# I-Mihara/BioDemuX.jl

Hardware: AMD Instinct MI355X
Metric: reads/s demultiplexed (150 bp, 96 barcodes, :semiglobal) at 1/2/4/8 MI355X (higher is better)
Workload: dtype i32

## Files before the change

### biodemux.jl_amd/csrc/bdx_sweep_col.h

```cpp
#pragma once
#include <stdint.h>

#if defined(__HIPCC__)
#define BDX_COL_FN __host__ __device__ __forceinline__
#else
#define BDX_COL_FN inline
#endif

#define BDX_COL_FIELD_MASK 0x1C1C1C1Cu

BDX_COL_FN uint32_t bdx_col_junk(const int nv) { return nv >= 8 ? 0u : (nv <= 0 ? 0x44444444u : (0x44444444u << (4 * nv))); }

BDX_COL_FN void bdx_col_fields(const uint32_t A, const uint32_t mask, uint32_t &ev, uint32_t &od) {
    ev = (A << 2) & mask;
    od = (A >> 2) & mask;
}
BDX_COL_FN uint32_t bdx_col_field(const uint32_t ev, const uint32_t od, const int k) { return (((k & 1) ? od : ev) >> (8 * (k >> 1))) & 0xFFu; }

BDX_COL_FN int bdx_col_score_carry(uint32_t &Ph, uint32_t &Mh, int score) {
#if defined(__has_builtin) && __has_builtin(__builtin_addc)
    uint32_t cp, cm;
    Ph = __builtin_addc(Ph, Ph, 0u, &cp);
    Mh = __builtin_addc(Mh, Mh, 0u, &cm);
#else
    const uint64_t p2 = (uint64_t)Ph + Ph, m2 = (uint64_t)Mh + Mh;
    const uint32_t cp = (uint32_t)(p2 >> 32), cm = (uint32_t)(m2 >> 32);
    Ph = (uint32_t)p2;
    Mh = (uint32_t)m2;
#endif
    score += (int)cp;
    score -= (int)cm;
    return score;
}

BDX_COL_FN uint32_t bdx_col_dbl(uint32_t x) {
#if defined(__HIP_DEVICE_COMPILE__)
    asm("v_add_u32 %0, %0, %0" : "+v"(x));
    return x;
#else
    return x + x;
#endif
}

template <bool TRACK, bool ADD = false>
BDX_COL_FN uint32_t sweep_step(const uint32_t Eq, uint32_t &Pv, uint32_t &Mv, int &score, int &best) {
    const uint32_t Xv = Eq | Mv;
    const uint32_t ep = Eq & Pv;
    const uint32_t Xh = ((ep + Pv) ^ Pv) | Eq;
    uint32_t Ph = Mv | ~(Xh | Pv);
    uint32_t Mh = Pv & Xh;
    if (TRACK) {
        score = bdx_col_score_carry(Ph, Mh, score);
    } else {
        Ph = ADD ? bdx_col_dbl(Ph) : Ph + Ph;
        Mh = ADD ? bdx_col_dbl(Mh) : Mh + Mh;
    }
    Pv = Mh | ~(Xv | Ph);
    Mv = Ph & Xv;
    if (TRACK) best = score < best ? score : best;
    return ep;
}
```

### biodemux.jl_amd/csrc/bdx_wave_kernel.h

```cpp
#pragma once

#include <atomic>

#include <cstdio>
#include <cstdlib>

#include "bdx_core.h"
#include "bdx_read_index.h"
#include "bdx_sweep_col.h"

#define BDX_BAD_PLAN() (getenv("BDX_TRACE_LAUNCH") ? (void)fprintf(stderr, "[bdx] launch refused at %s:%d\n", __FILE__, __LINE__) : (void)0, hipErrorInvalidValue)

namespace {

struct WaveArgs {
    double max_error_rate, min_delta;
    int counts_stride2;
    uint32_t rix_mul;
    const uint8_t *seq;
    const long long *off;
    long long n_reads;
    BdxDevOut out;
    unsigned long long *counts;
    int hist_entries;
// ... 31 lines not shown
    int vps, vps_inv;
    int max_len;
    int win_sfe, win_so, win_efe, win_eo;
    int cpr;
    int cpr_inv;
    int hq_cap, sq_cap;
    int ngroups;
    int scan_gpr, scan_gpr_inv;
    int cand_area;
    int ranged;
    BdxDevPass dpass[2];
    const uint32_t *idmap;
    const unsigned int *n_dev;
    uint32_t req;
    int dbg;
};

typedef const __attribute__((address_space(4))) WaveArgs *KArgs;
__device__ __forceinline__ KArgs kargs() {
    uint64_t p = (uint64_t)(uintptr_t)__builtin_amdgcn_kernarg_segment_ptr();
    asm volatile("" : "+s"(p));
    return (KArgs)(uintptr_t)p;
}

enum : uint32_t {
    REQ_BC1 = 1u, REQ_BC2 = 2u, REQ_KS = 4u, REQ_KE = 8u, REQ_PSTART = 16u, REQ_PEND = 32u, REQ_PRAW = 64u, REQ_PBC = 128u,
    REQ_PSCORE = 256u, REQ_PDELTA = 512u, REQ_COUNTS = 1024u,
    REQ_TIER = 2048u, REQ_DELTA = 4096u,
    REQ_PASS = REQ_PSTART | REQ_PEND | REQ_PRAW | REQ_PBC | REQ_PSCORE | REQ_PDELTA
};

#ifdef BDX_TUNING
#define BDX_DBG(bit) (a.dbg & (bit))
#else
#define BDX_DBG(bit) 0
#endif

typedef unsigned int u32x2 __attribute__((ext_vector_type(2)));
typedef unsigned int u32x3 __attribute__((ext_vector_type(3)));

#define WAVE_SYNC()                                          \
    do {                                                     \
        __builtin_amdgcn_fence(__ATOMIC_RELEASE, "wavefront"); \
        __builtin_amdgcn_wave_barrier();                     \
        __builtin_amdgcn_fence(__ATOMIC_ACQUIRE, "wavefront"); \
    } while (0)

template <bool EXACT, bool DOT>
__device__ __forceinline__ void pack16(const u32x4 v, uint32_t &p2, uint32_t &nlo, uint32_t &nhi, uint32_t &sad, const uint32_t m7 = 0x07070707u,
                                       const uint32_t m3 = 0x03030303u) {
    constexpr uint32_t CODE_LO = 0x03020100u, CODE_HI = 0x04040404u;
    constexpr uint32_t EXP_LO = 0x47544341u , EXP_HI = 0x4E000000u ;
    uint32_t u[4], t2[4];
#pragma unroll
    for (int w = 0; w < 4; ++w) {
        const uint32_t x = v[w];
        const uint32_t sel = (x >> 1) & m7;
        uint32_t n4 = __builtin_amdgcn_perm(CODE_HI, CODE_LO, sel);
        const uint32_t e = __builtin_amdgcn_perm(EXP_HI, EXP_LO, sel);
        if (EXACT) {
            const uint32_t d = x ^ e;
            const uint32_t y = (((d & 0x7F7F7F7Fu) + 0x7F7F7F7Fu) | d) & 0x80808080u;
            const uint32_t m = (y >> 7) * 0xFFu;
            n4 = (n4 & ~m) | (m & 0x04040404u);
        } else {
            sad = __builtin_amdgcn_sad_u8(x, e, sad);
        }
        u[w] = n4 | (n4 >> 4);
        if (DOT) {
            t2[w] = __builtin_amdgcn_udot4(sel & m3, 0x40100401u, 0u, false);
        } else {
            const uint32_t t6 = (x & 0x06060606u) << 5;
            const uint32_t a = t6 | (t6 << 6);
            t2[w] = a | (a << 12);
        }
    }
    nlo = __builtin_amdgcn_perm(u[1], u[0], 0x06040200u);
    nhi = __builtin_amdgcn_perm(u[3], u[2], 0x06040200u);
    const uint32_t lo = __builtin_amdgcn_perm(t2[1], t2[0], DOT ? 0x0C0C0400u : 0x0C0C0703u);
    const uint32_t hi = __builtin_amdgcn_perm(t2[3], t2[2], DOT ? 0x04000C0Cu : 0x07030C0Cu);
    p2 = lo | hi;
}

__device__ __forceinline__ void lds_read8(uint32_t (&d)[8], const uint32_t (&addr)[8]) {
#pragma unroll
    for (int i = 0; i < 8; ++i) asm volatile("ds_read_b32 %0, %1" : "=v"(d[i]) : "v"(addr[i]) : "memory");
}
__device__ __forceinline__ void lds_wait8(uint32_t (&d)[8]) {
    asm volatile("s_waitcnt lgkmcnt(0)"
                 : "+v"(d[0]), "+v"(d[1]), "+v"(d[2]), "+v"(d[3]), "+v"(d[4]), "+v"(d[5]), "+v"(d[6]), "+v"(d[7])
                 :
                 : "memory");
}

__device__ __forceinline__ int wave_cols(const int rem) {
    int x = 0;
#pragma unroll
    for (int bit = 16; bit > 0; bit >>= 1)
        if (__builtin_amdgcn_ballot_w64(rem > x + bit)) x += bit;
    return x + 1;
}

template <int TF, int TRACKW, bool COLS>
__device__ __forceinline__ void sweep_block(const uint32_t A0, const uint32_t A1, const uint32_t A2, const uint32_t A3,
                                            const uint32_t pbase, uint32_t &Pv, uint32_t &Mv, int &score, int &best, const int kk1,
                                            uint32_t &inm, uint32_t &inm2, const int nc) {
    const int ngr = COLS ? (nc + 7) >> 3 : nc;
    const uint32_t A[4] = {A0, A1, A2, A3};
    uint32_t Eq[2][8];
    uint32_t fmask = BDX_COL_FIELD_MASK;
    if (COLS) asm("" : "+v"(fmask));
    const auto issue = [&](const int h) __attribute__((always_inline)) {
        uint32_t addr[8];
        if (COLS) {
            uint32_t ev, od;
            bdx_col_fields(A[h], fmask, ev, od);
            asm volatile("" : "+v"(ev), "+v"(od));
#pragma unroll
            for (int jj = 0; jj < 8; ++jj) addr[jj] = pbase + bdx_col_field(ev, od, jj);
        } else {
#pragma unroll
            for (int jj = 0; jj < 8; ++jj) addr[jj] = pbase + (__builtin_amdgcn_ubfe(A[h], 4 * jj, 3) << 2);
        }
        lds_read8(Eq[h & 1], addr);
    };
    issue(0);
    inm = 0u;
    inm2 = 0u;
#pragma unroll
    for (int h = 0; h < 4; ++h) {
        if (h >= ngr) break;
        lds_wait8(Eq[h & 1]);
        if (h < 3 && h + 1 < ngr) issue(h + 1);
#pragma unroll
        for (int jj = 0; jj < 8; ++jj) {
            const int j = 8 * h + jj;
            if (COLS && jj > 0 && j >= nc) break;
            if (j < TF) {
                sweep_step<false, COLS>(Eq[h & 1][jj], Pv, Mv, score, best);
            } else {
                if (j == TF && TF > 0) score = __builtin_popcount(Pv) - __builtin_popcount(Mv);
                const int best_before = best;
                const uint32_t ep = sweep_step<true, COLS>(Eq[h & 1][jj], Pv, Mv, score, best);
                if (TRACKW == 1) inm = __builtin_amdgcn_alignbit(inm, (uint32_t)(score - kk1), 31);
                if (TRACKW >= 2) inm = __builtin_amdgcn_alignbit(inm, (uint32_t)(score - best_before), 31);
                if (TRACKW >= 3) inm2 = __builtin_amdgcn_alignbit(inm2, ep, 31);
            }
        }
    }
    const int ran = COLS ? nc : 8 * ngr;
    if (TRACKW && ran < 32) inm <<= 32 - ran;
    if (TRACKW >= 3 && ran < 32) inm2 <<= 32 - ran;
}

template <bool REVA>
__device__ __forceinline__ void anchored_block(const uint32_t A0, const uint32_t A1, const uint32_t A2, const uint32_t A3, const uint32_t pbase,
                                               const uint32_t rows, const uint32_t lowbit, uint32_t &Pv, uint32_t &Mv, int &score, const int d,
                                               uint32_t &eqm, uint32_t &inm2, const int ngr) {
    const uint32_t A[4] = {A0, A1, A2, A3};
    uint32_t Eq[2][8];
    const auto issue = [&](const int h) __attribute__((always_inline)) {
        uint32_t addr[8];
#pragma unroll
        for (int jj = 0; jj < 8; ++jj) addr[jj] = pbase + (__builtin_amdgcn_ubfe(A[h], 4 * jj, 3) << 2);
        lds_read8(Eq[h & 1], addr);
    };
// ... 54 lines not shown
    const uint32_t req = a.req;
    static_assert(!WINM || (!PAIRS && !SPLIT && KEND == 0 && GEN), "window mode: the non-split single-seed kernel");
    constexpr bool SCAT = PAIRS || WINM;
    constexpr bool CARRY = PAIRS && !SPLIT && !MG && KB <= 4;
    const uint32_t idmask = (CARRY && a.carry_ent != nullptr) ? 0x3FFFFFFFu : 0xFFFFFFFFu;
    const long long n_reads = (SCAT && a.n_dev) ? (long long)(unsigned int)__builtin_amdgcn_readfirstlane((int)*a.n_dev) : a.n_reads;

    size_t o = 0;
    auto take = [&](size_t bytes) -> LDS unsigned char * {
        LDS unsigned char *p = smem + o;
        o = (o + bytes + 31) & ~(size_t)31;
        return p;
    };
    LDS unsigned char *bm = take((size_t)a.bm_bytes);
    LDS uint16_t *rnk = (LDS uint16_t *)take(PAIRS ? 0 : (size_t)a.bm_bytes / 2);
    LDS uint32_t *ent = (LDS uint32_t *)take((size_t)a.n_ent * 4);
    LDS uint32_t *peq = (LDS uint32_t *)take((size_t)B * 36);
    LDS uint32_t *peqr = (LDS uint32_t *)take(KREV ? (size_t)B * 36 : 0);
    LDS uint32_t *meta = (LDS uint32_t *)take((size_t)B * 4);
    LDS uint32_t *settle = (LDS uint32_t *)take((size_t)B * 4);
    LDS int *hist = (LDS int *)take((size_t)a.hist_entries * 4);
    LDS unsigned char *wbase = smem + o + (size_t)wv * (size_t)a.per_wave;
    constexpr int O_FB = 0;
    constexpr int O_RID = O_FB + ((RW + 1) * 4 + 15) / 16 * 16;
    constexpr int O_RMK = O_RID + NREC * 4;
    constexpr int O_SLOTS = O_RMK + NREC * 4;
    constexpr int O_SCNT = O_SLOTS + RW * 16;
    constexpr int O_FLAG = O_SCNT + RW * 4;
    constexpr int O_WCL1 = O_FLAG + RW * 4;
    constexpr int O_LBUF = O_WCL1 + RW * 4;
    constexpr int O_RL = O_LBUF + 64 * 4;
    constexpr int O_GID = O_RL + (SCAT ? RW * 4 : 0);
    constexpr int O_TN = O_GID + (SCAT ? RW * 4 : 0);
    constexpr int O_SG4 = O_TN + ((WINM || PAIRS) ? RW * 4 : 0);
    constexpr int O_SGID = O_SG4 + (SCAT ? 2 * RW * 16 : 0);
    constexpr int O_STN = O_SGID + (SCAT ? 2 * RW * 4 : 0);
    constexpr int O_IMG2 = O_STN + ((WINM || PAIRS) ? 2 * RW * 4 : 0) + (SCAT ? 16 : 0);
    const int nvec_cap = a.span_cap >> 4;
    LDS int *fb = (LDS int *)(wbase + O_FB);
    LDS uint32_t *rid = (LDS uint32_t *)(wbase + O_RID);
    LDS uint32_t *rmk = (LDS uint32_t *)(wbase + O_RMK);
    LDS uint32_t *slots = (LDS uint32_t *)(wbase + O_SLOTS);
    LDS int *scnt = (LDS int *)(wbase + O_SCNT);
    LDS int *flag = (LDS int *)(wbase + O_FLAG);
    LDS int *wcl1 = (LDS int *)(wbase + O_WCL1);
    LDS uint32_t *lbuf = (LDS uint32_t *)(wbase + O_LBUF);
    LDS int *rl = (LDS int *)(wbase + O_RL);
    LDS uint32_t *gid = (LDS uint32_t *)(wbase + O_GID);
    LDS int *tn = (LDS int *)(wbase + O_TN);
    LDS u32x4 *sg4 = (LDS u32x4 *)(wbase + O_SG4);
    LDS uint32_t *sgid = (LDS uint32_t *)(wbase + O_SGID);
    LDS int *stn = (LDS int *)(wbase + O_STN);
    LDS uint32_t *img2 = (LDS uint32_t *)(wbase + O_IMG2);
    LDS uint32_t *img4 = img2 + ((nvec_cap + 2 + 3) & ~3);
    LDS uint32_t *hq = img4 + ((2 * nvec_cap + 6 + 3) & ~3);
    LDS uint32_t *recq = hq + HQ;
    const int cwt = a.cw[0] + a.cw[1];
    LDS uint32_t *cand = recq + SQ;
    LDS int *wwin = (LDS int *)(cand + RW * a.cand_area);
    const auto win_lo = [&](const int t, const bool second) -> int { return ranged ? wwin[(second ? 2 : 0) * RW + t] : 0; };
    const auto win_hi = [&](const int t, const bool second, const int n) -> int { return ranged ? wwin[(second ? 3 : 1) * RW + t] : n; };

    for (int i = tid; i < a.bm_bytes / 4; i += blockDim.x) ((LDS uint32_t *)bm)[i] = ((const uint32_t *)a.bitmap)[i];
    if (!PAIRS) {
        for (int i = tid; i < a.bm_bytes / 8; i += blockDim.x) ((LDS uint32_t *)rnk)[i] = ((const uint32_t *)a.rank)[i];
        for (int i = tid; i < a.n_ent; i += blockDim.x) ent[i] = a.ent[i];
    }
    if (SCAT && lane < 4) img2[lane - 4] = 0u;
    for (int i = tid; i < B * 9; i += blockDim.x) peq[i] = a.peq8[i];
    if (KREV)
        for (int i = tid; i < B * 9; i += blockDim.x) peqr[i] = a.peq8r[i];
    for (int i = tid; i < B; i += blockDim.x) {
        meta[i] = a.meta[i];
        settle[i] = a.settle[i];
    }
    for (int i = tid; i < a.hist_entries; i += blockDim.x) hist[i] = 0;
    __syncthreads();

    const uint32_t peq_base = (uint32_t)(uintptr_t)peq;
    const uint32_t peqr_base = (uint32_t)(uintptr_t)peqr;
    const int ntiles = (int)((n_reads + RW - 1) / RW);

    const int nwaves = (int)(gridDim.x * (blockDim.x >> 6));
    int tile = (int)(blockIdx.x * (blockDim.x >> 6)) + wv;
    struct Geo {
        long long span0;
        uintptr_t g0a;
        int head, total, nvec, nr;
        bool ok;
    };
    const auto geometry = [&](const int t, const long long ov) -> Geo {
        Geo g;
        const long long r0 = (long long)t * RW;
        g.nr = (int)(n_reads - r0 < RW ? n_reads - r0 : RW);
        const uint32_t ov_lo = (uint32_t)ov, ov_hi = (uint32_t)(ov >> 32);
        g.span0 = (long long)(((unsigned long long)__builtin_amdgcn_readlane(ov_hi, 0) << 32) | (uint32_t)__builtin_amdgcn_readlane(ov_lo, 0));
        const long long span1 = (long long)(((unsigned long long)__builtin_amdgcn_readlane(ov_hi, g.nr) << 32) | (uint32_t)__builtin_amdgcn_readlane(ov_lo, g.nr));
        const uintptr_t g0 = (uintptr_t)(a.seq + g.span0);
        g.g0a = g0 & ~(uintptr_t)15;
        g.head = (int)(g0 - g.g0a);
        const long long need = (span1 - g.span0) + g.head;
        g.ok = need + 16 <= (long long)a.span_cap && need <= (long long)NV * 1024;
        g.total = g.ok ? (int)need : 0;
        g.nvec = (g.total + 15) >> 4;
        return g;
    };
    typedef long long ll2a __attribute__((ext_vector_type(2), aligned(8)));
    struct ScatOff {
        long long o0;
        int len;
    };
    const auto load_scat = [&](const int t, const uint32_t id) -> ScatOff {
        const long long r0 = (long long)t * RW;
        ScatOff so{0, -1};
        if (SCAT && t < ntiles && r0 + lane < n_reads && lane < RW) {
            const ll2a o = *(const ll2a __attribute__((address_space(1))) *)(a.off + (CARRY ? (id & idmask) : id));
            so.o0 = o[0];
            const long long l = o[1] - o[0];
            so.len = (l >= 0 && l < (1LL << 30)) ? (int)l : -1;
        }
        return so;
    };
    struct ScatGeo {
        uintptr_t abase;
        int head, nv, len;
    };
    const auto scat_geo = [&](const ScatOff &so) -> ScatGeo {
        ScatGeo g{0, 0, 0, -1};
        if (so.len >= 0) {
            int wlo = 0, wlen = so.len;
            bool ok = true;
            if (WINM) {
                const int n = so.len;
                const int sx = a.win_sfe ? n + a.win_so : a.win_so, ex = a.win_efe ? n + a.win_eo : a.win_eo;
                const int first = sx > 1 ? sx : 1;
                int last = ex < n ? ex : n;
                if (last < first) last = first - 1;
                ok = n > 0 && first <= last;
                wlo = ok ? first - 1 : 0;
                wlen = ok ? last - first + 1 : 0;
            }
            const uintptr_t ad = (uintptr_t)a.seq + (uintptr_t)so.o0 + (uintptr_t)wlo;
            g.head = (int)(ad & 15);
            g.abase = ad - (uintptr_t)g.head;
            const int nv = (g.head + wlen + 15) >> 4;
            if (ok && nv <= a.vps && (WINM || so.len <= a.max_len)) {
                g.nv = nv;
                g.len = wlen;
            }
        }
        return g;
    };
    const auto load_offsets = [&](const int t) -> long long {
        const long long r0 = (long long)t * RW;
        const long long left = n_reads - r0;
        const int cnt = t < ntiles ? (int)(left < RW ? left : RW) : -1;
        if (SCAT) return 0;
        const uintptr_t bp = (uintptr_t)(a.off + r0);
        const uint32_t blo = __builtin_amdgcn_readfirstlane((uint32_t)bp), bhi = __builtin_amdgcn_readfirstlane((uint32_t)(bp >> 32));
        const long long *base = (const long long *)(((uintptr_t)bhi << 32) | blo);
        return lane <= cnt ? base[lane] : 0;
    };
    const auto load_gid = [&](const int t) -> uint32_t {
        const long long r0 = (long long)t * RW;
        return (SCAT && t < ntiles && r0 + lane < n_reads && lane < RW) ? (a.idmap ? a.idmap[r0 + lane] : (uint32_t)(r0 + lane)) : 0u;
    };
    const auto rlen = [&](const int t) -> int { return SCAT ? rl[t] : fb[t + 1] - fb[t]; };
// ... 37 lines not shown
    int lcnt = 0;
    const auto flush_list = [&]() {
        if (lcnt > 0) {
            WAVE_SYNC();
            unsigned int basek = 0;
            if (lane == 0) basek = atomicAdd(a.list_count, (unsigned int)lcnt);
            basek = (unsigned int)__builtin_amdgcn_readfirstlane((int)basek);
            if (lane < lcnt) a.list[basek + lane] = lbuf[lane];
            WAVE_SYNC();
            lcnt = 0;
        }
    };
    long long ov = load_offsets(tile);
    Geo geo{};
    uint32_t iv_next = load_gid(tile + nwaves), iv_after = load_gid(tile + 2 * nwaves);
    ScatOff so_next = load_scat(tile + nwaves, iv_next);
    int par = 0;
    const auto scat_tile = [&](const int t) -> Geo {
        Geo g{};
        const long long r0 = (long long)t * RW;
        g.nr = (int)(n_reads - r0 < RW ? n_reads - r0 : RW);
        g.ok = true;
        g.nvec = g.nr * a.vps;
        g.total = g.nvec << 4;
        return g;
    };
    if (tile < ntiles) {
        if (SCAT) {
            geo = scat_tile(tile);
            const uint32_t iv0 = load_gid(tile);
            stash_scat(0, load_scat(tile, iv0), iv0);
            load_bytes_scat(0, geo.nr);
        } else {
            geo = geometry(tile, ov);
            load_bytes(geo);
        }
    }
    long long ov_next = load_offsets(tile + nwaves);

    while (tile < ntiles) {
        const long long r0 = (long long)tile * RW;
        const int nr = geo.nr;
        const bool tile_ok = geo.ok;
        const int total = geo.total, nvec = geo.nvec;

        if (!SCAT && lane <= nr) fb[lane] = tile_ok ? geo.head + (int)(ov - geo.span0) : 0;
        if (lane < RW) {
            scnt[lane] = 0;
            flag[lane] = 0;
            if (SCAT) {
                const u32x4 e = sg4[par * RW + lane];
                const int slen = (int)e[3];
                fb[lane] = lane * a.slot + (int)(e[2] >> 8);
                rl[lane] = lane < nr ? slen : 0;
                gid[lane] = sgid[par * RW + lane] & idmask;
                if (CARRY) tn[lane] = a.carry_ent != nullptr ? (int)(sgid[par * RW + lane] >> 30) : 0;
                if (WINM) {
                    tn[lane] = stn[par * RW + lane];
                    if (lane < nr && slen < 0) flag[lane] = 1;
                }
            }
            wcl1[lane] = 0;
            if (CARRY && lane < nr) {
                const int st = tn[lane];
                if (st == 1) {
                    slots[lane * 4] = (uint32_t)stn[par * RW + lane];
                    scnt[lane] = 1;
                } else if (st == 2) {
                    cand[lane * 4] = (uint32_t)stn[par * RW + lane];
                    wcl1[lane] = 1;
                }
            }
            if (SPLIT)
                for (int w = 0; w < cwt; ++w) cand[lane * cwt + w] = 0u;
        }

        uint32_t m7 = 0x07070707u, m3 = 0x03030303u;
        if (LEAN) asm volatile("" : "+v"(m7), "+v"(m3));
#pragma unroll
        for (int u = 0; u < NV; ++u) {
            const int k = 64 * u + lane;
            if (64 * u < nvec) {
                uint32_t p2 = 0, nlo = 0, nhi = 0, sad = 0;
                if (k < nvec && !BDX_DBG(32)) pack16<false, LEAN>(v[u], p2, nlo, nhi, sad, m7, m3);
                if (__builtin_amdgcn_ballot_w64(sad != 0)) {
                    if (sad != 0) pack16<true, LEAN>(v[u], p2, nlo, nhi, sad, m7, m3);
                }
                if (k < nvec) {
                    img2_lane[64 * u] = p2;
                    *(LDS u32x2 *)(img4_lane + 128 * u) = u32x2{nlo, nhi};
                }
            }
        }
        const int tile_next = tile + nwaves;
        Geo geo_next{};
        if (tile_next < ntiles) {
            if (SCAT) {
                geo_next = scat_tile(tile_next);
                stash_scat(par ^ 1, so_next, iv_next);
                load_bytes_scat(par ^ 1, geo_next.nr);
            } else {
                geo_next = geometry(tile_next, ov_next);
                load_bytes(geo_next);
            }
        }
        const long long ov_after = load_offsets(tile_next + nwaves);
        const ScatOff so_after = load_scat(tile_next + nwaves, iv_after);
        const uint32_t iv_after2 = load_gid(tile_next + 2 * nwaves);
        WAVE_SYNC();

        if (ranged && lane < RW) {
            const int n = lane < nr ? rlen(lane) : 0;
            bool known = true;
            const KArgs ka = kargs();
#pragma unroll
            for (int p = 0; p < 2; ++p) {
                PassWindow w{1, 0, 0, 0};
                BdxDevPass dp;
                __builtin_memcpy(&dp, (const void *)&ka->dpass[p], sizeof dp);
                const bool ok = (p == 0 || a.B0 < B) && lane < nr && pass_window(dp, n, w);
                wwin[(2 * p) * RW + lane] = ok ? w.first - 1 : 0;
                wwin[(2 * p + 1) * RW + lane] = ok ? w.last : 0;
                if (p == 0 || a.B0 < B) known = known && ok && n > 0 && w.max_start >= n && w.min_end <= 1;
            }
            if (!SPLIT && !known && lane < nr) flag[lane] = 1;
        }
        if (ranged) WAVE_SYNC();

        int ulen = 0;
        {
            const int my = (!SCAT && lane < nr) ? fb[lane + 1] - fb[lane] : 0;
            const int l0 = __builtin_amdgcn_readfirstlane(my);
            ulen = (l0 > (LEAN ? 1 : 0) && !__builtin_amdgcn_ballot_w64(lane < nr && my != l0)) ? l0 : 0;
        }

        const auto sweep_lane = [&](bool valid, const int t, const int b, const int lo, const int hi) __attribute__((always_inline)) {
            const uint32_t mt = meta[b];
            const int mm = (int)(mt & 255u), kk = (int)((mt >> 8) & 255u);
            valid = valid && hi > lo && !BDX_DBG(2);
            const int ncol = valid ? hi - lo : 0;
            uint32_t Pv = mm >= 32 ? 0xFFFFFFFFu : (((1u << mm) - 1u) << (32 - mm));
            uint32_t Mv = 0;
            int score = mm, best = 0x7FFFFFFF;
            const bool second_b = GEN && b >= a.B0;
            const int trim_b = KEND ? (second_b ? a.trim1 : a.trim0) : 0;
            const bool rev = KREV && trim_b == 3;
            const uint32_t pbase = (rev ? peqr_base : peq_base) + (uint32_t)b * 36u;
            const int sb0 = fb[t] + lo;
            const int se0 = fb[t] + hi - 32;
            int e_lo = 0, e_hi = -1;
            uint32_t sflag = 0u;
            for (int blk = 0;; ++blk) {
                const int rem = ncol - 32 * blk;
                if (!__builtin_amdgcn_ballot_w64(rem > 0)) break;
                const int sb = rev ? se0 - 32 * blk : sb0 + 32 * blk;
                const int d0 = sb >> 3, shb = (sb & 7) * 4;
                uint32_t W[5];
#pragma unroll
                for (int u = 0; u < 5; ++u) W[u] = (valid && (!KREV || rem > 0)) ? img4[d0 + u] : 0u;
                uint32_t A[4];
#pragma unroll
                for (int u = 0; u < 4; ++u) A[u] = __builtin_amdgcn_alignbit(W[u + 1], W[u], shb);
                if (KREV) {
                    uint32_t R[4];
#pragma unroll
                    for (int u = 0; u < 4; ++u) {
                        const uint32_t y = __builtin_amdgcn_perm(0u, A[3 - u], 0x00010203u);
                        R[u] = ((y & 0x0F0F0F0Fu) << 4) | ((y >> 4) & 0x0F0F0F0Fu);
                    }
#pragma unroll
                    for (int u = 0; u < 4; ++u) A[u] = rev ? R[u] : A[u];
                }
#pragma unroll
                for (int u = 0; u < 4; ++u) {
                    const int nv = rem - 8 * u;
                    const uint32_t junk = nv >= 8 ? 0u : (nv <= 0 ? 0x44444444u : (0x44444444u << (4 * nv)));
                    A[u] |= junk;
                }
                uint32_t inm = 0u, inm2 = 0u;
                const int ncw = LEAN ? wave_cols(rem)
                                     : (__builtin_amdgcn_ballot_w64(rem > 24) ? 4 : (__builtin_amdgcn_ballot_w64(rem > 16) ? 3 : (__builtin_amdgcn_ballot_w64(rem > 8) ? 2 : 1)));
                if (blk == 0)
                    sweep_block<TF, (SPLIT ? 1 : KEND ? 1 + KEND : 0), LEAN>(A[0], A[1], A[2], A[3], pbase, Pv, Mv, score, best, kk + 1, inm, inm2, ncw);
                else
                    sweep_block<0, (SPLIT ? 1 : KEND ? 1 + KEND : 0), LEAN>(A[0], A[1], A[2], A[3], pbase, Pv, Mv, score, best, kk + 1, inm, inm2, ncw);
                if (KEND && !SPLIT) {
                    inm &= rem >= 32 ? 0xFFFFFFFFu : (rem <= 0 ? 0u : ~((1u << (32 - rem)) - 1u));
                    if (inm) {
                        const int tz = (int)__builtin_ctz(inm);
                        e_hi = 32 * blk + 31 - tz;
                        sflag = (inm2 >> tz) & 1u;
                    }
                }
                if (SPLIT) {
                    inm &= rem >= 32 ? 0xFFFFFFFFu : (rem <= 0 ? 0u : ~((1u << (32 - rem)) - 1u));
                    if (inm) {
                        if (e_hi < 0) e_lo = 32 * blk + (int)__builtin_clz(inm);
                        e_hi = 32 * blk + 31 - (int)__builtin_ctz(inm);
                    }
                }
            }
            if (valid && best <= kk) {
                if (SPLIT) {
                    const int pass = b >= a.B0 ? 1 : 0;
                    const int bl = b - (pass ? a.B0 : 0);
                    __hip_atomic_fetch_or(&cand[t * cwt + (pass ? a.cw[0] : 0) + (bl >> 5)], 1u << (bl & 31), __ATOMIC_RELAXED, __HIP_MEMORY_SCOPE_WORKGROUP);
                    const int kx = __hip_atomic_fetch_add(pass ? &wcl1[t] : &scnt[t], 1, __ATOMIC_RELAXED, __HIP_MEMORY_SCOPE_WORKGROUP);
                    if (kx < BDX_WCAP && e_hi >= 0) {
                        const int jf_abs = lo + 1;
                        const int lb = !a.sg ? mm - 1 : ((pass ? a.short_lb[1] : a.short_lb[0]) ? mm + kk : 2 * (mm + kk) + 1);
                        const size_t rg = PAIRS ? (size_t)gid[t] : (size_t)(r0 + t);
                        uint32_t *dst = (pass ? a.wins_out[1] : a.wins_out[0]) + (rg * BDX_WCAP + kx) * 3;
                        dst[0] = (uint32_t)bl;
                        dst[1] = (uint32_t)(jf_abs + e_lo - lb);
                        dst[2] = (uint32_t)(jf_abs + e_hi);
                    }
                } else {
                    const bool second = GEN && b >= a.B0;
                    const int bl = second ? b - a.B0 : b;
                    const int ks = __hip_atomic_fetch_add(second ? &wcl1[t] : &scnt[t], 1, __ATOMIC_RELAXED, __HIP_MEMORY_SCOPE_WORKGROUP);
                    uint32_t pkey = 0u;
                    if (KEND && (trim_b == 5 || (KALN && trim_b == 0 && a.need_tb))) pkey = (uint32_t)(lo + e_hi + 1);
                    if (KREV && rev) {
                        const int pstar = hi - 1 - e_hi;
                        const int origin = (sflag == 0u && pstar <= win_lo(t, second)) ? 0 : pstar + (int)sflag;
                        pkey = 0xFFFFu - (uint32_t)origin;
                    }
                    if (ks < 4) (second ? cand : slots)[t * 4 + ks] = KEND ? (((uint32_t)bl << 22) | ((uint32_t)best << 16) | pkey) : (((uint32_t)bl << 8) | (uint32_t)best);
                }
            }
        };
        int nhq = 0;
        bool hq_over = false;
        const auto drain = [&]() __attribute__((always_inline)) {
            WAVE_SYNC();
            hq_over = hq_over || nhq > HQ;
            const int nh = BDX_DBG(4) ? 0 : (nhq < HQ ? nhq : HQ);
            for (int s0 = 0; s0 < nh; s0 += 64) {
                const int k = s0 + lane;
                bool valid = k < nh;
                const uint32_t h = valid ? hq[k] : 0u;
                const int b = (int)(h & 511u), t = (int)((h >> 9) & 15u), wd = (int)((h >> 13) & 15u), dlo = (int)(h >> 17) - 64;
                const uint32_t mt = meta[b];
                const int mm = (int)(mt & 255u), kk = (int)((mt >> 8) & 255u);
                valid = valid && kk != 255;
                const int n = rl[t];
                const int sp = KB >= 8 ? (int)(mt >> 24) : kk;
                const int dr = dlo - (fb[t] - t * a.slot);
                int lo = dr - sp, hi = dr + wd + mm + sp;
                const int wlo = win_lo(t, b >= a.B0), whi = win_hi(t, b >= a.B0, n);
                lo = lo < wlo ? wlo : lo;
                hi = hi > whi ? whi : hi;
                sweep_lane(valid, t, b, lo, hi);
            }
            nhq = 0;
            WAVE_SYNC();
        };

        if constexpr (PAIRS) {
            constexpr int PL = KB == 9 ? 3 : 4;
            constexpr int P = KB == 8 ? 6 : KB == 9 ? 8 : KB + 2;
            constexpr int ND = KB >= 8 ? 0 : KB;
            constexpr int ESTRIDE = NW <= 2 ? 8 : 16;
            constexpr int TSTRIDE = (1 << (2 * PL)) * ESTRIDE;
            constexpr int XLO = -8 - ND;
            constexpr int NX = 16 + ND + PL * (P - 1);
            static_assert(7 + PL * (P - 1) + PL - 1 <= 31, "the keys of a chunk come out of three words of the 2-bit image");
            uint32_t amask = ((1u << (2 * PL)) - 1u) * ESTRIDE;
            asm volatile("" : "+v"(amask));
            const int s16 = a.vps;
            const int items = BDX_DBG(8) ? 0 : nr * a.cpr;
            for (int i0 = 0; i0 < items; i0 += 64) {
                const int i = i0 + lane;
                const bool on = i < items;
                const int t = on ? (int)(((uint32_t)i * (uint32_t)a.cpr_inv) >> 16) : 0;
                const int c = on ? i - t * a.cpr : 0;
                uint32_t ad[NX];
                uint32_t Fl[NW], dmw[NW];
                const int gword = t * s16 + c;
                uint32_t wm1 = 0u, w0 = 0u, w1 = 0u;
                const auto keys = [&]() __attribute__((always_inline)) {
                    wm1 = img2[gword - 1];
                    w0 = img2[gword];
                    w1 = img2[gword + 1];
                };
                const auto key_addr = [&](const int xi) __attribute__((always_inline)) -> uint32_t {
                    const int bit = 2 * (XLO + xi + 16) - (ESTRIDE == 16 ? 4 : 3);
                    static_assert(2 * (XLO + 16) - 4 >= 0, "the first key's bits start inside the first word");
                    const int wi = bit >> 5, sh = bit & 31;
                    const uint32_t lo = wi == 0 ? wm1 : (wi == 1 ? w0 : w1);
                    const uint32_t hi = wi == 0 ? w0 : (wi == 1 ? w1 : 0u);
                    return __builtin_amdgcn_alignbit(hi, lo, sh) & amask;
                };
                const auto diagonals = [&](const uint32_t gbase) __attribute__((always_inline)) {
                    uint32_t Ah[ND > 0 ? ND : 1][NW];
#pragma unroll
                    for (int j = -ND; j < 16; ++j) {
#pragma unroll
                        for (int xi = (j == -ND ? 0 : j + ND + PL * (P - 1)); xi <= j + ND + PL * (P - 1); ++xi) ad[xi] = key_addr(xi);
                        uint32_t H[P][NW];
#pragma unroll
                        for (int tt = 0; tt < P; ++tt) {
                            const uint32_t ea = ad[j - 8 + PL * tt - XLO] + gbase + (uint32_t)(tt * TSTRIDE);
                            if constexpr (NW == 1) {
                                H[tt][0] = *(const LDS uint32_t *)(bm + ea);
                            } else if constexpr (NW == 2) {
                                const u32x2 x = *(const LDS u32x2 *)(bm + ea);
                                H[tt][0] = x[0];
                                H[tt][1] = x[1];
                            } else {
                                const u32x4 x = *(const LDS u32x4 *)(bm + ea);
                                H[tt][0] = x[0];
                                H[tt][1] = x[1];
                                H[tt][2] = x[2];
                                if constexpr (NW == 4) H[tt][3] = x[3];
                            }
                        }
#pragma unroll
                        for (int w = 0; w < NW; ++w) {
                            uint32_t once = H[0][w] | H[1][w];
                            uint32_t twice = H[0][w] & H[1][w];
#pragma unroll
                            for (int tt = 2; tt < P; ++tt) {
                                if (j >= 0) twice |= once & H[tt][w];
                                once |= H[tt][w];
                            }
                            if (j >= 0) {
                                uint32_t F = twice;
                                if constexpr (ND > 0) {
                                    uint32_t near = Ah[0][w];
#pragma unroll
                                    for (int u = 1; u < ND; ++u) near |= Ah[u][w];
                                    F |= once & near;
                                }
                                Fl[w] |= F;
                                dmw[w] = (dmw[w] << 1) | (F != 0u ? 1u : 0u);
// ... 300 lines not shown
                            idx = e >> 16;
                            bool inwin = true;
                            if (ranged) {
                                const bool second_b = (int)(e & 2047u) - 1 >= a.B0;
                                inwin = p >= wwin[(second_b ? 2 : 0) * RW + t] && p + q <= wwin[(second_b ? 3 : 1) * RW + t];
                            }
                            if (inwin) {
                                const uint32_t pb = e & 2047u;
                                const int kk = (int)((meta[pb - 1u] >> 8) & 255u);
                                const int diag = p - (int)((e >> 11) & 31u);
                                const uint32_t mine = pb | ((uint32_t)(diag + 64) << 16);
                                int rs = (int)((pb + (uint32_t)(diag >> 3)) & (RCAP - 1));
                                bool placed = false;
                                for (int tries = 0; tries < RCAP && !placed; ++tries) {
                                    LDS uint32_t *id = rid + t * RCAP + rs;
                                    uint32_t old = *id;
                                    bool opened = false;
                                    if (old == 0u) {
                                        uint32_t expect = 0u;
                                        __hip_atomic_compare_exchange_strong(id, &expect, mine, __ATOMIC_RELAXED, __ATOMIC_RELAXED, __HIP_MEMORY_SCOPE_WORKGROUP);
                                        opened = expect == 0u;
                                        old = opened ? mine : expect;
                                    }
                                    const int dd = diag - ((int)(old >> 16) - 64);
                                    if ((old & 0xFFFFu) == pb && dd >= -kk && dd <= kk) {
                                        __hip_atomic_fetch_or(&rmk[t * RCAP + rs], 1u << (dd + kk), __ATOMIC_RELAXED, __HIP_MEMORY_SCOPE_WORKGROUP);
                                        placed = true;
                                        if (opened) {
                                            if (new0 < 0)
                                                new0 = t * RCAP + rs;
                                            else if (new1 < 0)
                                                new1 = t * RCAP + rs;
                                            else {
                                                if (flag[t] != 1) flag[t] = 2;
                                                rid[t * RCAP + rs] = 0u;
                                                rmk[t * RCAP + rs] = 0u;
                                            }
                                        }
                                    }
                                    rs = (rs + 1) & (RCAP - 1);
                                }
                                if (!placed && flag[t] != 1) flag[t] = 2;
                            }
                        } while (idx != 0u);
                    }
                }
#pragma unroll
                for (int layer = 0; layer < 2; ++layer) {
                    const int nw = layer == 0 ? new0 : new1;
                    const unsigned long long mk = __builtin_amdgcn_ballot_w64(nw >= 0);
                    if (mk) {
                        const int kq = ns + (int)__builtin_amdgcn_mbcnt_hi((uint32_t)(mk >> 32), __builtin_amdgcn_mbcnt_lo((uint32_t)mk, 0u));
                        if (nw >= 0) {
                            if (kq < SQ) {
                                recq[kq] = (uint32_t)nw;
                            } else {
                                if (flag[nw / RCAP] != 1) flag[nw / RCAP] = 2;
                                rid[nw] = 0u;
                                rmk[nw] = 0u;
                            }
                        }
                        ns += (int)__builtin_popcountll(mk);
                    }
                }
            }
        }
        ns = ns < SQ ? ns : SQ;
        WAVE_SYNC();

        if constexpr (!PAIRS)
        for (int s0 = 0; s0 < ns; s0 += 64) {
            const int k = s0 + lane;
            bool valid = k < ns;
            const uint32_t rslot = valid ? recq[k] : 0u;
            const uint32_t id = valid ? rid[rslot] : 0u;
            const uint32_t dmk = valid ? rmk[rslot] : 0u;
            if (valid) {
                rid[rslot] = 0u;
                rmk[rslot] = 0u;
            }
            valid = valid && id != 0u && dmk != 0u;
            const int t = (int)(rslot / RCAP), b = valid ? (int)(id & 0xFFFFu) - 1 : 0;
            int lo = 0, hi = 0;
            if (valid) {
                const uint32_t mt = meta[b];
                const int mm = (int)(mt & 255u), kk = (int)((mt >> 8) & 255u);
                const int d0 = (int)(id >> 16) - 64;
                const int dmin = d0 + __builtin_ctz(dmk) - kk, dmax = d0 + (31 - __builtin_clz(dmk)) - kk;
                const int n = rlen(t);
                constexpr int SLACK = (!SPLIT && KEND == 0) ? 0 : 1;
                lo = dmin - kk - SLACK;
                hi = dmax + mm + kk + SLACK;
                int wlo = 0, whi = n;
                if (ranged) {
                    wlo = wwin[(b >= a.B0 ? 2 : 0) * RW + t];
                    whi = wwin[(b >= a.B0 ? 3 : 1) * RW + t];
                }
                lo = lo < wlo ? wlo : lo;
                hi = hi > whi ? whi : hi;
            }
            sweep_lane(valid, t, b, lo, hi);
        }
        WAVE_SYNC();
        if (SPLIT || !PAIRS) {
            unsigned long long fm = !tile_ok ? 0ull
                                    : SPLIT  ? __builtin_amdgcn_ballot_w64(lane < nr && (flag[lane] != 0 || !hq_ok))
                                             : ((hq_ok && !(a.dbg & (1 << 30))) ? __builtin_amdgcn_ballot_w64(lane < nr && flag[lane] == 2) : 0ull);
            while (fm) {
                const int t = (int)__builtin_ctzll(fm);
                fm &= fm - 1ull;
                if (lane == 0) {
                    scnt[t] = 0;
                    wcl1[t] = 0;
                    flag[t] = 0;
                    if (SPLIT)
                        for (int w = 0; w < cwt; ++w) cand[t * cwt + w] = 0u;
                }
                WAVE_SYNC();
                const int n = rlen(t);
                for (int b0 = 0; b0 < B; b0 += 64) {
                    const int b = b0 + lane < B ? b0 + lane : 0;
                    const bool valid = b0 + lane < B && ((meta[b] >> 8) & 255u) != 255u;
                    sweep_lane(valid, t, b, win_lo(t, b >= a.B0), win_hi(t, b >= a.B0, n));
                }
                WAVE_SYNC();
            }
        }

        if (SPLIT) {
            if (lane < nr && !BDX_DBG(1)) {
                const long long rid_g = PAIRS ? (long long)gid[lane] : r0 + lane;
                const bool usable = tile_ok && !flag[lane] && (!PAIRS || rl[lane] >= 0);
#pragma unroll
                for (int pass = 0; pass < 2; ++pass) {
                    if (pass == 1 && a.cw[1] == 0) break;
                    const int cwp = pass ? a.cw[1] : a.cw[0];
                    uint32_t *dst = (pass ? a.cand_out[1] : a.cand_out[0]) + rid_g * cwp;
                    for (int w = 0; w < cwp; ++w) dst[w] = usable ? cand[lane * cwt + (pass ? a.cw[0] : 0) + w] : 0xFFFFFFFFu;
                    const int c = pass ? wcl1[lane] : scnt[lane];
                    (pass ? a.wcnt_out[1] : a.wcnt_out[0])[rid_g] = (unsigned char)((usable && c <= BDX_WCAP) ? c : 255);
                }
            }
            WAVE_SYNC();
            tile = tile_next;
            geo = geo_next;
            ov = ov_next;
            ov_next = ov_after;
            so_next = so_after;
            iv_next = iv_after;
            iv_after = iv_after2;
            par ^= 1;
            continue;
        }

        uint32_t rq = req;
        asm volatile("" : "+s"(rq));
        const bool active = lane < nr;
        const long long ridx = SCAT ? (long long)gid[lane < RW ? lane : 0] : r0 + lane;
        Verdict vd{0, 0, -1, -1};
        PassOut p1{0, 0, -1, -1, -1, __builtin_inf(), __builtin_inf()}, p2{2, 0, -1, -1, -1, __builtin_inf(), __builtin_inf()};
        bool done = false;
        uint32_t cst = 0u, centry = 0u;
        if (active && tile_ok && hq_ok && !BDX_DBG(1)) {
            const int n = WINM ? tn[lane] : rlen(lane);
            const int cnt = scnt[lane], cnt1 = dual ? wcl1[lane] : 0;
            const bool simple = (rq & REQ_PASS) == 0u;
            const bool tiered = (rq & REQ_TIER) != 0u;
            if (simple && !KALN && !flag[lane] && cnt <= 1 && cnt1 <= 1 && n >= 1) {
                done = true;
                int pos1 = 0, pos2 = 0;
                const int sbit = (rq & REQ_DELTA) ? 16 : 0;
                uint32_t soff = (uint32_t)((B + 7) & ~7);
                asm volatile("" : "+s"(soff));
                const LDS uint32_t *const settle_w = meta + soff;
                bool settled_all = true;
                if (cnt == 1) {
                    const uint32_t e = slots[lane * 4];
                    const int bb = KEND ? (int)(e >> 22) : (int)(e >> 8), d = KEND ? (int)((e >> 16) & 63u) : (int)(e & 255u);
                    pos1 = (int)(e & 0xFFFFu);
                    const int dmax = (int)((meta[bb] >> 16) & 255u);
                    vd.bc1 = (dmax != 255 && d <= dmax) ? bb + 1 : 0;
                    settled_all = tiered && vd.bc1 > 0 && ((settle_w[bb] >> (d + sbit)) & 1u) != 0u;
                } else {
                    vd.bc1 = 0;
                    settled_all = false;
                }
                const bool s1_settled = settled_all;
                vd.bc2 = 0;
                if (dual && vd.bc1 > 0) {
                    int bc2v = 0;
                    bool s2 = false;
                    if (cnt1 == 1) {
                        const uint32_t e = cand[lane * 4];
                        const int bb = KEND ? (int)(e >> 22) : (int)(e >> 8), d = KEND ? (int)((e >> 16) & 63u) : (int)(e & 255u), g = a.B0 + bb;
                        pos2 = (int)(e & 0xFFFFu);
                        const int dmax = (int)((meta[g] >> 16) & 255u);
                        bc2v = (dmax != 255 && d <= dmax) ? bb + 1 : 0;
                        s2 = tiered && bc2v > 0 && ((settle_w[g] >> (d + sbit)) & 1u) != 0u;
                    }
                    settled_all = settled_all && s2;
                    vd.bc2 = bc2v;
                    if (bc2v == 0) vd.bc1 = 0;
                    if (bc2v == 0) vd.bc2 = 0;
                }
                if (tiered) done = settled_all;
                if (!PAIRS && tiered && dual && a.carry_ent != nullptr && !settled_all) {
// ... 440 lines not shown
```

Baseline: 10.18 billion.

## Streamline lean-path packing, junk masking, meta reuse and tile interleave

Result: faster. 10.39 billion, median of 6 (+2.1%).

```diff
diff --git a/biodemux.jl_amd/csrc/bdx_sweep_col.h b/biodemux.jl_amd/csrc/bdx_sweep_col.h
--- a/biodemux.jl_amd/csrc/bdx_sweep_col.h
+++ b/biodemux.jl_amd/csrc/bdx_sweep_col.h
@@ -10,6 +10,14 @@
 #define BDX_COL_FIELD_MASK 0x1C1C1C1Cu
 
 BDX_COL_FN uint32_t bdx_col_junk(const int nv) { return nv >= 8 ? 0u : (nv <= 0 ? 0x44444444u : (0x44444444u << (4 * nv))); }
+
+BDX_COL_FN uint32_t bdx_col_junk_word(const int rem, const int u) {
+    int nv = rem - 8 * u;
+    nv = nv < 0 ? 0 : (nv > 8 ? 8 : nv);
+    return (uint32_t)(0x44444444ull << (4 * nv));
+}
+
+BDX_COL_FN uint32_t bdx_col_pv0(const int m) { return 0xFFFFFFFFu << ((32 - m) & 31); }
 
 BDX_COL_FN void bdx_col_fields(const uint32_t A, const uint32_t mask, uint32_t &ev, uint32_t &od) {
     ev = (A << 2) & mask;
diff --git a/biodemux.jl_amd/csrc/bdx_wave_kernel.h b/biodemux.jl_amd/csrc/bdx_wave_kernel.h
--- a/biodemux.jl_amd/csrc/bdx_wave_kernel.h
+++ b/biodemux.jl_amd/csrc/bdx_wave_kernel.h
@@ -137,6 +137,40 @@
     p2 = lo | hi;
 }
 
+__device__ __forceinline__ void pack16_lean(const u32x4 v, const bool live, uint32_t &p2, uint32_t &nlo, uint32_t &nhi, const uint32_t m7, const uint32_t m3) {
+    constexpr uint32_t CODE_LO = 0x03020100u, CODE_HI = 0x04040404u;
+    constexpr uint32_t EXP_LO = 0x47544341u, EXP_HI = 0x4E000000u;
+    uint32_t sel[4], n4[4], e[4], sad = 0;
+#pragma unroll
+    for (int w = 0; w < 4; ++w) {
+        sel[w] = (v[w] >> 1) & m7;
+        n4[w] = __builtin_amdgcn_perm(CODE_HI, CODE_LO, sel[w]);
+        e[w] = __builtin_amdgcn_perm(EXP_HI, EXP_LO, sel[w]);
+        sad = __builtin_amdgcn_sad_u8(v[w], e[w], sad);
+    }
+    const bool bad = live && sad != 0;
+    if (__builtin_amdgcn_ballot_w64(bad)) {
+        if (bad) {
+#pragma unroll
+            for (int w = 0; w < 4; ++w) {
+                const uint32_t d = v[w] ^ e[w];
+                const uint32_t y = (((d & 0x7F7F7F7Fu) + 0x7F7F7F7Fu) | d) & 0x80808080u;
+                const uint32_t m = (y >> 7) * 0xFFu;
+                n4[w] = (n4[w] & ~m) | (m & 0x04040404u);
+            }
+        }
+    }
+    uint32_t u[4], t2[4];
+#pragma unroll
+    for (int w = 0; w < 4; ++w) {
+        u[w] = n4[w] | (n4[w] >> 4);
+        t2[w] = __builtin_amdgcn_udot4(sel[w] & m3, 0x40100401u, 0u, false);
+    }
+    nlo = __builtin_amdgcn_perm(u[1], u[0], 0x06040200u);
+    nhi = __builtin_amdgcn_perm(u[3], u[2], 0x06040200u);
+    p2 = __builtin_amdgcn_perm(t2[1], t2[0], 0x0C0C0400u) | __builtin_amdgcn_perm(t2[3], t2[2], 0x04000C0Cu);
+}
+
 __device__ __forceinline__ void lds_read8(uint32_t (&d)[8], const uint32_t (&addr)[8]) {
 #pragma unroll
     for (int i = 0; i < 8; ++i) asm volatile("ds_read_b32 %0, %1" : "=v"(d[i]) : "v"(addr[i]) : "memory");
@@ -357,7 +391,7 @@
     const int ntiles = (int)((n_reads + RW - 1) / RW);
 
     const int nwaves = (int)(gridDim.x * (blockDim.x >> 6));
-    int tile = (int)(blockIdx.x * (blockDim.x >> 6)) + wv;
+    int tile = LEAN ? wv * (int)gridDim.x + (int)blockIdx.x : (int)(blockIdx.x * (blockDim.x >> 6)) + wv;
     struct Geo {
         long long span0;
         uintptr_t g0a;
@@ -561,9 +595,13 @@
             const int k = 64 * u + lane;
             if (64 * u < nvec) {
                 uint32_t p2 = 0, nlo = 0, nhi = 0, sad = 0;
-                if (k < nvec && !BDX_DBG(32)) pack16<false, LEAN>(v[u], p2, nlo, nhi, sad, m7, m3);
-                if (__builtin_amdgcn_ballot_w64(sad != 0)) {
-                    if (sad != 0) pack16<true, LEAN>(v[u], p2, nlo, nhi, sad, m7, m3);
+                if constexpr (LEAN) {
+                    if (!BDX_DBG(32)) pack16_lean(v[u], k < nvec, p2, nlo, nhi, m7, m3);
+                } else {
+                    if (k < nvec && !BDX_DBG(32)) pack16<false, LEAN>(v[u], p2, nlo, nhi, sad, m7, m3);
+                    if (__builtin_amdgcn_ballot_w64(sad != 0)) {
+                        if (sad != 0) pack16<true, LEAN>(v[u], p2, nlo, nhi, sad, m7, m3);
+                    }
                 }
                 if (k < nvec) {
                     img2_lane[64 * u] = p2;
@@ -613,12 +651,12 @@
             ulen = (l0 > (LEAN ? 1 : 0) && !__builtin_amdgcn_ballot_w64(lane < nr && my != l0)) ? l0 : 0;
         }
 
-        const auto sweep_lane = [&](bool valid, const int t, const int b, const int lo, const int hi) __attribute__((always_inline)) {
-            const uint32_t mt = meta[b];
+        const auto sweep_lane = [&](bool valid, const int t, const int b, const int lo, const int hi, const uint32_t mt_in) __attribute__((always_inline)) {
+            const uint32_t mt = LEAN ? mt_in : meta[b];
             const int mm = (int)(mt & 255u), kk = (int)((mt >> 8) & 255u);
             valid = valid && hi > lo && !BDX_DBG(2);
             const int ncol = valid ? hi - lo : 0;
-            uint32_t Pv = mm >= 32 ? 0xFFFFFFFFu : (((1u << mm) - 1u) << (32 - mm));
+            uint32_t Pv = LEAN ? bdx_col_pv0(mm) : (mm >= 32 ? 0xFFFFFFFFu : (((1u << mm) - 1u) << (32 - mm)));
             uint32_t Mv = 0;
             int score = mm, best = 0x7FFFFFFF;
             const bool second_b = GEN && b >= a.B0;
@@ -650,11 +688,20 @@
 #pragma unroll
                     for (int u = 0; u < 4; ++u) A[u] = rev ? R[u] : A[u];
                 }
-#pragma unroll
-                for (int u = 0; u < 4; ++u) {
-                    const int nv = rem - 8 * u;
-                    const uint32_t junk = nv >= 8 ? 0u : (nv <= 0 ? 0x44444444u : (0x44444444u << (4 * nv)));
-                    A[u] |= junk;
+                if constexpr (LEAN) {
+                    if (!__builtin_amdgcn_ballot_w64(valid && rem < 24)) {
+                        A[3] |= bdx_col_junk_word(rem, 3);
+                    } else {
+#pragma unroll
+                        for (int u = 0; u < 4; ++u) A[u] |= bdx_col_junk_word(rem, u);
+                    }
+                } else {
+#pragma unroll
+                    for (int u = 0; u < 4; ++u) {
+                        const int nv = rem - 8 * u;
+                        const uint32_t junk = nv >= 8 ? 0u : (nv <= 0 ? 0x44444444u : (0x44444444u << (4 * nv)));
+                        A[u] |= junk;
+                    }
                 }
                 uint32_t inm = 0u, inm2 = 0u;
                 const int ncw = LEAN ? wave_cols(rem)
@@ -730,7 +777,7 @@
                 const int wlo = win_lo(t, b >= a.B0), whi = win_hi(t, b >= a.B0, n);
                 lo = lo < wlo ? wlo : lo;
                 hi = hi > whi ? whi : hi;
-                sweep_lane(valid, t, b, lo, hi);
+                sweep_lane(valid, t, b, lo, hi, mt);
             }
             nhq = 0;
             WAVE_SYNC();
@@ -1197,8 +1244,10 @@
             valid = valid && id != 0u && dmk != 0u;
             const int t = (int)(rslot / RCAP), b = valid ? (int)(id & 0xFFFFu) - 1 : 0;
             int lo = 0, hi = 0;
+            uint32_t mt_rec = 0u;
             if (valid) {
                 const uint32_t mt = meta[b];
+                if (LEAN) mt_rec = mt;
                 const int mm = (int)(mt & 255u), kk = (int)((mt >> 8) & 255u);
                 const int d0 = (int)(id >> 16) - 64;
                 const int dmin = d0 + __builtin_ctz(dmk) - kk, dmax = d0 + (31 - __builtin_clz(dmk)) - kk;
@@ -1214,7 +1263,7 @@
                 lo = lo < wlo ? wlo : lo;
                 hi = hi > whi ? whi : hi;
             }
-            sweep_lane(valid, t, b, lo, hi);
+            sweep_lane(valid, t, b, lo, hi, mt_rec);
         }
         WAVE_SYNC();
         if (SPLIT || !PAIRS) {
@@ -1236,7 +1285,7 @@
                 for (int b0 = 0; b0 < B; b0 += 64) {
                     const int b = b0 + lane < B ? b0 + lane : 0;
                     const bool valid = b0 + lane < B && ((meta[b] >> 8) & 255u) != 255u;
-                    sweep_lane(valid, t, b, win_lo(t, b >= a.B0), win_hi(t, b >= a.B0, n));
+                    sweep_lane(valid, t, b, win_lo(t, b >= a.B0), win_hi(t, b >= a.B0, n), LEAN ? meta[b] : 0u);
                 }
                 WAVE_SYNC();
             }
```
